# twndus/YelpRecommendation

Hardware: NVIDIA B200
Metric: ngcf_bpr_train_triples_per_sec (higher is better)
Workload: dtype f32

## Files before the change

yelprecommendation_b200/csrc/common.cuh:

```cuda
#pragma once
#include <cuda_runtime.h>
#include <cooperative_groups.h>
#include <stdint.h>
#include "../../include/yelprec_b200.h"

namespace cg = cooperative_groups;

#define YR_CHECK_LAUNCH()                                   \
  do {                                                      \
    cudaError_t e__ = cudaGetLastError();                   \
    if (e__ != cudaSuccess) return (int)e__;                \
  } while (0)

#define YR_CUDA(call)                                       \
  do {                                                      \
    cudaError_t e__ = (call);                               \
    if (e__ != cudaSuccess) return (int)e__;                \
  } while (0)

int yr_eval_exact_launch(const float* Uemb, int64_t nU, const float* Vt, int64_t ldt, int64_t nI, int d,
                         const int64_t* eval_uid, int64_t n_eval, const int32_t* mask_ptr,
                         const int32_t* mask_idx, const int32_t* act_ptr, const int32_t* act_idx,
                         const int32_t* act_nuniq, const double* inv_log2, int K, int64_t* topk_out,
                         float* topk_score, double* user_metrics, int32_t* err, const int32_t* row_list,
                         const int32_t* n_rows_dev, yr_stream stream, void* ws = nullptr, size_t ws_bytes = 0);
int yr_eval_reduce_launch(const double* user_metrics, const int32_t* act_ptr, const int32_t* act_nuniq,
                          int64_t n_eval, double* metric_sums, yr_stream stream);

int yr_ngcf_dense_fwd_tc_launch_d(int d, const float* E, const float* LE, const float* W1, const float* W2, float slope,
                                  int64_t n, float* Eout, cudaStream_t s, const int32_t* row_list = nullptr,
                                  const int32_t* row_count = nullptr, int64_t row_cap = 0, int reserve_sms = 0);
int yr_ngcf_dense_bwd_tc_launch(int d, const float* E, const float* LE, const float* En, const float* Gn, const float* W1,
                                const float* W2, float slope, int64_t n, float* G, float* T, float* ws, int* n_parts,
                                cudaStream_t s, const int32_t* row_list = nullptr, const int32_t* row_count = nullptr,
                                int64_t row_cap = 0, int reserve_sms = 0);
int yr_spmm_csr_rows(const yr_csr* A, int d, const float* X, float* Y, const int32_t* row_flag, cudaStream_t s);

namespace yr {

constexpr int kWarp = 32;
constexpr unsigned kFull = 0xffffffffu;

__device__ __forceinline__ float warp_sum(float v) {
#pragma unroll
  for (int o = 16; o > 0; o >>= 1) v += __shfl_xor_sync(kFull, v, o);
  return v;
}
__device__ __forceinline__ double warp_sum_d(double v) {
#pragma unroll
  for (int o = 16; o > 0; o >>= 1) v += __shfl_xor_sync(kFull, v, o);
  return v;
}

__device__ __forceinline__ void grid_sync(cg::grid_group& grid) {
  __syncwarp();
  grid.sync();
  __syncwarp();
}
// ... 181 lines not shown
```

yelprecommendation_b200/csrc/ngcf.cu:

```cuda
#include <stdlib.h>
#include "common.cuh"

namespace yr {

__device__ __forceinline__ void fma2(float2& acc, float a, const float2 b) { acc = __ffma2_rn(make_float2(a, a), b, acc); }

template <int D>
struct DenseCfg {
  static constexpr int kThreads = 256;
  static constexpr int kColGroups = D / 4;
  static constexpr int kRowGroups = kThreads / kColGroups;
  static constexpr int TM = 4 * kRowGroups;
  static constexpr int RO = D / kRowGroups;
  static constexpr size_t kSmemFwd = (size_t)(2 * D * TM + 2 * D * D) * sizeof(float);
  static constexpr size_t kSmemBwd = (size_t)(3 * TM * D + 2 * D * D) * sizeof(float);
  static_assert(D == 32 || D == 64 || D == 128, "dense transforms: D in {32, 64, 128}");
};

template <int D>
__global__ void __launch_bounds__(256)
ngcf_dense_fwd_kernel(const float* __restrict__ E, const float* __restrict__ LE,
                      const float* __restrict__ W1, const float* __restrict__ W2, float slope,
                      int64_t n, float* __restrict__ Eout) {
  using C = DenseCfg<D>;
// ... 436 lines not shown
                                 float slope, float* E_next, int dense_mode, yr_stream stream) {
  if (!E || !LE || !W1 || !W2 || !E_next || n < 0 || !mode_ok(dense_mode)) return YR_ERR_BAD_ARG;
  if (d != 32 && d != 64 && d != 128) return YR_ERR_BAD_DIM;
  if (n == 0) return YR_OK;
  if (fwd_tc(dense_mode) && (d == 64 || d == 128))
    return yr_ngcf_dense_fwd_tc_launch_d(d, E, LE, W1, W2, slope, n, E_next, (cudaStream_t)stream, nullptr, nullptr, 0,
                                         reserve_of(dense_mode));
  switch (d) {
    case 32: return dense_fwd_fp32_launch<32>(n, E, LE, W1, W2, slope, E_next, (cudaStream_t)stream);
    case 64: return dense_fwd_fp32_launch<64>(n, E, LE, W1, W2, slope, E_next, (cudaStream_t)stream);
    default: return dense_fwd_fp32_launch<128>(n, E, LE, W1, W2, slope, E_next, (cudaStream_t)stream);
  }
}

extern "C" int yr_ngcf_layer_fwd(const yr_csr* L, int d, const float* E, const float* W1, const float* W2,
                                 float slope, float* E_next, float* LE_save, int dense_mode, yr_stream stream) {
  if (!L || !E || !W1 || !W2 || !E_next || !LE_save || L->n_rows <= 0 || !mode_ok(dense_mode)) return YR_ERR_BAD_ARG;
  if (d != 32 && d != 64 && d != 128) return YR_ERR_BAD_DIM;
  int rc = yr_spmm_csr(L, d, E, LE_save, 0, stream);
  if (rc) return rc;
  return yr_ngcf_dense_fwd(d, L->n_rows, E, LE_save, W1, W2, slope, E_next, dense_mode, stream);
}

extern "C" size_t yr_ngcf_layer_bwd_ws_bytes(int d) {
  return (size_t)yr_sm_count() * kBwdCtasPerSm * 2 * (size_t)d * d * sizeof(float);
}

static int dense_bwd_launch(int d, int64_t n, const float* E, const float* LE, const float* E_next, const float* G_next,
                            const float* W1, const float* W2, float slope, float* G, float* T, void* ws, size_t ws_bytes,
                            int dense_mode, cudaStream_t s, int* n_parts) {
  if (!E || !LE || !E_next || !G_next || !W1 || !W2 || !G || !T || !ws || n <= 0 || !mode_ok(dense_mode)) return YR_ERR_BAD_ARG;
  if (d != 32 && d != 64 && d != 128) return YR_ERR_BAD_DIM;
  if (ws_bytes < yr_ngcf_layer_bwd_ws_bytes(d)) return YR_ERR_WORKSPACE;
  if (bwd_tc(dense_mode) && (d == 64 || d == 128))
    return yr_ngcf_dense_bwd_tc_launch(d, E, LE, E_next, G_next, W1, W2, slope, n, G, T, (float*)ws, n_parts, s, nullptr, nullptr,
                                       0, reserve_of(dense_mode));
  switch (d) {
    case 32: return dense_bwd_fp32_launch<32>(n, E, LE, E_next, G_next, W1, W2, slope, G, T, (float*)ws, s, n_parts);
    case 64: return dense_bwd_fp32_launch<64>(n, E, LE, E_next, G_next, W1, W2, slope, G, T, (float*)ws, s, n_parts);
    default: return dense_bwd_fp32_launch<128>(n, E, LE, E_next, G_next, W1, W2, slope, G, T, (float*)ws, s, n_parts);
  }
}

static int dense_bwd_reduce(int d, const void* ws, int n_parts, float* dW1, float* dW2, cudaStream_t s) {
  const int len = 2 * d * d;
  reduce_partials_kernel<<<(len + 31) / 32, 256, 0, s>>>((const float*)ws, n_parts, len, dW1, dW2, d * d);
  YR_CHECK_LAUNCH();
  return YR_OK;
}

extern "C" int yr_ngcf_dense_bwd(int d, int64_t n, const float* E, const float* LE, const float* E_next,
                                 const float* G_next, const float* W1, const float* W2, float slope,
                                 float* G, float* T, float* dW1, float* dW2, void* ws, size_t ws_bytes,
                                 int dense_mode, yr_stream stream) {
  if (!dW1 || !dW2) return YR_ERR_BAD_ARG;
  int parts = 0;
  int rc = dense_bwd_launch(d, n, E, LE, E_next, G_next, W1, W2, slope, G, T, ws, ws_bytes, dense_mode, (cudaStream_t)stream,
                            &parts);
  if (rc) return rc;
// ... 42 lines not shown
    float4 t[VPT];
#pragma unroll
    for (int v = 0; v < VPT; ++v)
      t[v] = len ? reinterpret_cast<const float4*>(T + (int64_t)row * D)[sl * VPT + v] : make_float4(0.f, 0.f, 0.f, 0.f);
    for (int j0 = 0; j0 < maxlen; j0 += LPR) {
      const int j = j0 + sl;
      const int cc = (j < len) ? __ldg(A.col + s0 + j) : -1;
      const float aa = (j < len) ? __ldg(A.val + s0 + j) : 0.f;
      for (int q = 0; q < LPR && j0 + q < maxlen; ++q) {
        const int cq = __shfl_sync(kFull, cc, q, LPR);
        const float a = __shfl_sync(kFull, aa, q, LPR);
        if (cq >= 0) {
#pragma unroll
          for (int v = 0; v < VPT; ++v)
            atomicAdd(reinterpret_cast<float4*>(G + (int64_t)cq * D) + sl * VPT + v,
                      make_float4(a * t[v].x, a * t[v].y, a * t[v].z, a * t[v].w));
        }
      }
    }
  }
}
}

struct SideStream { cudaStream_t stream; cudaEvent_t fork, join; };
static SideStream* side_stream() {
  static SideStream pool[64];
  static int state[64];
  const char* e = getenv("YR_NGCF_SIDE_STREAM");
  if (e && e[0] == '0') return nullptr;
  int dev = 0;
  if (cudaGetDevice(&dev) != cudaSuccess || dev < 0 || dev >= 64) return nullptr;
  if (state[dev] == 0) {
    SideStream& x = pool[dev];
    const bool ok = cudaStreamCreateWithFlags(&x.stream, cudaStreamNonBlocking) == cudaSuccess &&
                    cudaEventCreateWithFlags(&x.fork, cudaEventDisableTiming) == cudaSuccess &&
                    cudaEventCreateWithFlags(&x.join, cudaEventDisableTiming) == cudaSuccess;
    state[dev] = ok ? 1 : -1;
  }
  return state[dev] == 1 ? &pool[dev] : nullptr;
}

static int rows_reduce(const yr_ngcf_state* st, int l, int parts, cudaStream_t s, SideStream* side);

static int ngcf_layer_bwd_rows(const yr_ngcf_state* st, int l, float slope, cudaStream_t s, SideStream* side) {
  const int d = st->d;
  using C = DenseCfg<64>;
  if (d != 64) return YR_ERR_BAD_DIM;
  if (bwd_tc(st->dense_mode) && st->row_list_cap >= 16384) {
    int parts = 0;
    int rc = yr_ngcf_dense_bwd_tc_launch(d, st->E[l], st->LE[l], st->E[l + 1], st->G[l + 1], st->W1[l], st->W2[l], slope,
                                         st->nU + st->nI, st->G[l], st->T, (float*)st->ws, &parts, s, st->row_list,
                                         st->row_count, st->row_list_cap);
    if (rc) return rc;
    rc = rows_reduce(st, l, parts, s, side);
    if (rc) return rc;
    const int64_t blocks_tc = ((int64_t)st->L.n_chunks + 15) / 16;
    spmm_scatter_rows_kernel<64><<<(unsigned)blocks_tc, 256, 0, s>>>(st->L, st->row_flag, st->T, st->G[l]);
    YR_CHECK_LAUNCH();
    return YR_OK;
  }
  int64_t grid = (st->row_list_cap + C::TM - 1) / C::TM;
  const int64_t cap = (int64_t)yr_sm_count() * kBwdCtasPerSm;
  if (grid > cap) grid = cap;
  if (grid < 1) grid = 1;
  static AttrOnce attr;
  { int rc_ = attr.set(ngcf_dense_bwd_kernel<64>, (int)C::kSmemBwd); if (rc_) return rc_; }
  ngcf_dense_bwd_kernel<64><<<(unsigned)grid, C::kThreads, C::kSmemBwd, s>>>(
      st->E[l], st->LE[l], st->E[l + 1], st->G[l + 1], st->W1[l], st->W2[l], slope, st->nU + st->nI, st->G[l], st->T,
      (float*)st->ws, st->row_list, st->row_count);
  YR_CHECK_LAUNCH();
  int rc = rows_reduce(st, l, (int)grid, s, side);
  if (rc) return rc;
  const int wpb = 8, cpw = 2;
  int64_t blocks = ((int64_t)st->L.n_chunks + wpb * cpw - 1) / (wpb * cpw);
  spmm_scatter_rows_kernel<64><<<(unsigned)blocks, 256, 0, s>>>(st->L, st->row_flag, st->T, st->G[l]);
// ... 153 lines not shown
}

static int train_step_body(const yr_ngcf_state* st, const yr_opt* opt, float slope,
                           const int64_t* uid, const int64_t* pos, const int64_t* neg, int64_t B,
                           float* step_loss, int prefix_done, yr_stream stream, bool* rows_armed) {
  int rc = ngcf_state_ok(st);
  if (rc) return rc;
  if (prefix_done < 0 || prefix_done > st->n_layers) return YR_ERR_BAD_ARG;
  if (!opt || !uid || !pos || !neg || B <= 0 || yr_csr_ok(&st->LT) || !st->T ||
      !st->E_dev || !st->G_dev || !st->ws || !st->loss)
    return YR_ERR_BAD_ARG;
  if (opt->kind < YR_OPT_SGD || opt->kind > YR_OPT_ADAMW) return YR_ERR_BAD_OPT;
  const int L = st->n_layers, d = st->d;
  const int64_t n = st->nU + st->nI;
  cudaStream_t s = (cudaStream_t)stream;
  SideStream* side = side_stream();
  for (int l = 0; l <= L; ++l)
    if (!st->G[l]) return YR_ERR_BAD_ARG;
  cudaStream_t ms = side ? side->stream : s;
  if (side) {
    YR_CUDA(cudaEventRecord(side->fork, s));
    YR_CUDA(cudaStreamWaitEvent(side->stream, side->fork, 0));
  }
  for (int l = 0; l <= L; ++l) YR_CUDA(cudaMemsetAsync(st->G[l], 0, sizeof(float) * (size_t)n * d, ms));
  const bool rows_path = st->row_flag && st->row_list && st->row_count && st->row_list_cap >= 3 * B && d == 64 &&
                         st->top_rows_mode != 0;
  if (rows_path) {
    touched_rows_kernel<<<(unsigned)((3 * B + 255) / 256), 256, 0, ms>>>(uid, pos, neg, B, st->nU, st->nI, st->row_flag,
                                                                        st->row_list, st->row_count);
    YR_CHECK_LAUNCH();
    *rows_armed = true;
  }
  if (side) YR_CUDA(cudaEventRecord(side->join, side->stream));
  if (rows_path && fwd_tc(st->dense_mode)) {
    for (int l = (prefix_done < L - 1 ? prefix_done : L - 1); l + 1 < L; ++l) {
      rc = yr_ngcf_layer_fwd(&st->L, d, st->E[l], st->W1[l], st->W2[l], slope, st->E[l + 1], st->LE[l], st->dense_mode,
                           stream);
      if (rc) return rc;
    }
    if (side) YR_CUDA(cudaStreamWaitEvent(s, side->join, 0));
    rc = yr_spmm_csr_rows(&st->L, d, st->E[L - 1], st->LE[L - 1], st->row_flag, s);
    if (rc) return rc;
    rc = yr_ngcf_dense_fwd_tc_launch_d(d, st->E[L - 1], st->LE[L - 1], st->W1[L - 1], st->W2[L - 1], slope, n, st->E[L], s,
                                       st->row_list, st->row_count, 3 * B);
    if (rc) return rc;
  } else {
    for (int l = prefix_done; l < L; ++l) {
      rc = yr_ngcf_layer_fwd(&st->L, d, st->E[l], st->W1[l], st->W2[l], slope, st->E[l + 1], st->LE[l], st->dense_mode,
                           stream);
      if (rc) return rc;
    }
  }
  if (side) YR_CUDA(cudaStreamWaitEvent(s, side->join, 0));
  rc = yr_ngcf_tail(st->E_dev, st->G_dev, L, st->nU, st->nI, d, uid, pos, neg, B, nullptr, nullptr, st->loss,
                    step_loss, st->err, stream);
  if (rc) return rc;
  bool reduce_pending = false;
  for (int l = L - 1; l >= 0; --l) {
    if (!st->dW1[l] || !st->dW2[l]) return YR_ERR_BAD_ARG;
    if (rows_path && l == L - 1) {
      rc = ngcf_layer_bwd_rows(st, l, slope, s, side);
      if (rc) return rc;
      reduce_pending = side != nullptr;
      cudaStream_t us = s;
      if (side) {
        YR_CUDA(cudaStreamWaitEvent(s, side->join, 0));
        reduce_pending = false;
        YR_CUDA(cudaEventRecord(side->fork, s));
        YR_CUDA(cudaStreamWaitEvent(side->stream, side->fork, 0));
        us = side->stream;
      }
      untouch_rows_kernel<<<(unsigned)((3 * B + 255) / 256), 256, 0, us>>>(st->row_flag, st->row_list, st->row_count);
      YR_CHECK_LAUNCH();
      YR_CUDA(cudaMemsetAsync(st->row_count, 0, sizeof(int32_t), us));
      *rows_armed = false;
      continue;
    }
    if (side && reduce_pending) { YR_CUDA(cudaStreamWaitEvent(s, side->join, 0)); reduce_pending = false; }
    int parts = 0;
    rc = dense_bwd_launch(d, n, st->E[l], st->LE[l], st->E[l + 1], st->G[l + 1], st->W1[l], st->W2[l], slope, st->G[l],
                          st->T, st->ws, st->ws_bytes, st->dense_mode, s, &parts);
    if (rc) return rc;
    if (side) {
      YR_CUDA(cudaEventRecord(side->fork, s));
      YR_CUDA(cudaStreamWaitEvent(side->stream, side->fork, 0));
      rc = dense_bwd_reduce(d, st->ws, parts, st->dW1[l], st->dW2[l], side->stream);
      if (rc) return rc;
      YR_CUDA(cudaEventRecord(side->join, side->stream));
      reduce_pending = true;
    } else {
      rc = dense_bwd_reduce(d, st->ws, parts, st->dW1[l], st->dW2[l], s);
      if (rc) return rc;
    }
    rc = yr_spmm_csr(&st->LT, d, st->T, st->G[l], 1, stream);
    if (rc) return rc;
  }
  if (side && reduce_pending) YR_CUDA(cudaStreamWaitEvent(s, side->join, 0));
  float *pp[2 * YR_NGCF_MAX_LAYERS + 1], *gg[2 * YR_NGCF_MAX_LAYERS + 1], *mm[2 * YR_NGCF_MAX_LAYERS + 1],
      *vv[2 * YR_NGCF_MAX_LAYERS + 1];
  int64_t nn[2 * YR_NGCF_MAX_LAYERS + 1];
  int cnt = 0;
  pp[cnt] = st->E[0]; gg[cnt] = st->G[0]; mm[cnt] = st->mE; vv[cnt] = st->vE; nn[cnt++] = n * d;
  for (int l = 0; l < L; ++l) {
    pp[cnt] = st->W1[l]; gg[cnt] = st->dW1[l]; mm[cnt] = st->mW1[l]; vv[cnt] = st->vW1[l]; nn[cnt++] = (int64_t)d * d;
// ... 39 lines not shown
```

yelprecommendation_b200/csrc/ngcf_tc.cu:

```cuda
#include <stdlib.h>
#include "tc_common.cuh"

namespace yr {

constexpr int kFwdThreads = 416;
constexpr int kFwdTM = 128;

template <int D>
struct FwdTc {
  static_assert(D == 64 || D == 128, "tensor-core forward: d in {64, 128}");
  static constexpr bool kBRes = (D == 64);
  static constexpr int kSlabs = D / 32;
  static constexpr uint32_t kABytes = 128 * 128;
  static constexpr uint32_t kBBytes = D * 128;
  static constexpr uint32_t kStage = 2 * kABytes + (kBRes ? 0u : 2 * kBBytes);
  static constexpr int kNst = kBRes ? 4 : 3;
  static constexpr uint32_t kRing = kNst * kStage;
  static constexpr uint32_t kBResBytes = kBRes ? (uint32_t)(2 * kSlabs * 2) * kBBytes : 0u;
  static constexpr uint32_t kEpiOff = kRing + kBResBytes;
  static constexpr uint32_t kEpiBytes = 4 * 32 * 256;
  static constexpr uint32_t kBarOff = kEpiOff + kEpiBytes;
  static constexpr size_t kSmem = (size_t)kBarOff + 256 + 1024;
  static constexpr uint32_t kTmemCols = 4 * D;
  static constexpr size_t kWsBytes = (size_t)(2 * kSlabs) * 2 * kBBytes;
// ... 7 lines not shown
               "l"(src), "r"(bytes), "r"(s2u(bar))
               : "memory");
}

template <int D>
__global__ void __launch_bounds__(256)
ngcf_split_weights_kernel(const float* __restrict__ W1, const float* __restrict__ W2, unsigned char* __restrict__ ws) {
  using C = FwdTc<D>;
  const int total = 2 * D * (D / 4);
  for (int idx = blockIdx.x * blockDim.x + threadIdx.x; idx < total; idx += gridDim.x * blockDim.x) {
    const int X = idx / (D * (D / 4)), rem = idx % (D * (D / 4));
    const int o = rem / (D / 4), c4 = rem % (D / 4), j = c4 >> 3, c = c4 & 7;
    float4 hi, lo;
    split4(__ldg(reinterpret_cast<const float4*>((X ? W2 : W1) + o * D) + c4), hi, lo);
    unsigned char* blk = ws + (size_t)(j * 2 + X) * 2 * C::kBBytes;
    const uint32_t off = sw_off(D, o, c);
    *reinterpret_cast<float4*>(blk + off) = hi;
    *reinterpret_cast<float4*>(blk + C::kBBytes + off) = lo;
  }
}

template <int D>
__global__ void __launch_bounds__(kFwdThreads, 1)
ngcf_dense_fwd_tc_kernel(const float* __restrict__ E, const float* __restrict__ LE, const float* __restrict__ W1,
                         const float* __restrict__ W2, const unsigned char* __restrict__ wsplit, float slope, int64_t n,
                         float* __restrict__ Eout, const int32_t* __restrict__ row_list,
                         const int32_t* __restrict__ row_count) {
  using C = FwdTc<D>;
  constexpr int kSlabs = C::kSlabs, kNst = C::kNst;
  constexpr uint32_t kABytes = C::kABytes, kBBytes = C::kBBytes, kStage = C::kStage;
  if (row_list) n = *row_count;
  extern __shared__ __align__(16) unsigned char smem_raw[];
  unsigned char* smem = smem_raw + ((1024u - (s2u(smem_raw) & 1023u)) & 1023u);
  unsigned char* ring = smem;
  unsigned char* bres = smem + C::kRing;
  uint64_t* bars = reinterpret_cast<uint64_t*>(smem + C::kBarOff);
  uint64_t* full = bars; uint64_t* empty = bars + kNst; uint64_t* d_full = bars + 2 * kNst; uint64_t* d_empty = d_full + 2;
  uint32_t* tmem_slot = reinterpret_cast<uint32_t*>(d_empty + 2);

  const int tid = threadIdx.x, lane = tid & 31, warp = tid >> 5;
  const int64_t n_tiles = (n + kFwdTM - 1) / kFwdTM;
  const int64_t my_tiles = (int64_t)blockIdx.x < n_tiles ? (n_tiles - blockIdx.x + gridDim.x - 1) / gridDim.x : 0;

  if (tid == 0) {
    for (int s = 0; s < kNst; ++s) { mbar_init(full + s, 1); mbar_init(empty + s, 1); }
    for (int a = 0; a < 2; ++a) { mbar_init(d_full + a, 1); mbar_init(d_empty + a, 128); }
    asm volatile("fence.mbarrier_init.release.cluster;" ::: "memory");
  }
  if (warp == 12) tmem_alloc(tmem_slot, C::kTmemCols);
  if constexpr (C::kBRes) {
    for (int idx = tid; idx < D * (D / 4); idx += kFwdThreads) {
      const int o = idx / (D / 4), c4 = idx % (D / 4), j = c4 >> 3, c = c4 & 7;
      const uint32_t off = sw_off(D, o, c);
      float4 hi, lo;
      split4(__ldg(reinterpret_cast<const float4*>(W1 + o * D) + c4), hi, lo);
      *reinterpret_cast<float4*>(bres + (size_t)((0 * kSlabs + j) * 2 + 0) * kBBytes + off) = hi;
      *reinterpret_cast<float4*>(bres + (size_t)((0 * kSlabs + j) * 2 + 1) * kBBytes + off) = lo;
      split4(__ldg(reinterpret_cast<const float4*>(W2 + o * D) + c4), hi, lo);
      *reinterpret_cast<float4*>(bres + (size_t)((1 * kSlabs + j) * 2 + 0) * kBBytes + off) = hi;
      *reinterpret_cast<float4*>(bres + (size_t)((1 * kSlabs + j) * 2 + 1) * kBBytes + off) = lo;
    }
  }
  asm volatile("fence.proxy.async.shared::cta;" ::: "memory");
  tc_fence_before();
  __syncthreads();
  tc_fence_after();
  const uint32_t tmem_base = *tmem_slot;
  const uint32_t idesc = (1u << 4) | (2u << 7) | (2u << 10) | ((uint32_t)(D >> 3) << 17) | ((uint32_t)(128 >> 4) << 24);

  if (warp < 8) {
    const int c = tid & 7, rb = tid >> 3;
    const int64_t n_items = my_tiles * kSlabs;
    uint32_t s = 0, ph = 0;
    constexpr int kPfTiles = 1;
    auto prefetch_tile = [&](int64_t ti) {
      if (row_list || ti >= my_tiles) return;
      const int64_t r0 = (blockIdx.x + ti * gridDim.x) * kFwdTM;
      const int64_t rows = (n - r0) < kFwdTM ? (n - r0) : kFwdTM;
      l2_prefetch_bulk(E + r0 * D, (uint32_t)(rows * D * 4));
      l2_prefetch_bulk(LE + r0 * D, (uint32_t)(rows * D * 4));
    };
    auto issue = [&](int64_t item, float4 (&e)[4], float4 (&le)[4]) {
      const int64_t tile = blockIdx.x + (item / kSlabs) * gridDim.x;
      const int j = (int)(item % kSlabs);
#pragma unroll
      for (int i = 0; i < 4; ++i) {
// ... 83 lines not shown
            o.z = o.z > 0.f ? o.z : o.z * slope; o.w = o.w > 0.f ? o.w : o.w * slope;
            *reinterpret_cast<float4*>(stg + lane * 256 + (((8 * half + k) ^ (lane & 15)) << 4)) = o;
          }
        }
        __syncwarp();
        {
#pragma unroll 4
          for (int i = 0; i < 16; ++i) {
            const int rr = 2 * i + (lane >> 4), c4 = lane & 15;
            const int64_t q = q0 + rr;
            const float4 o = *reinterpret_cast<const float4*>(stg + rr * 256 + ((c4 ^ (rr & 15)) << 4));
            if (q < n) {
              const int64_t row = row_list ? (int64_t)__ldg(row_list + q) : q;
              reinterpret_cast<float4*>(Eout + row * D + 64 * h)[c4] = o;
            }
          }
        }
        __syncwarp();
      }
      if (++acc == 2) { acc = 0; aph ^= 1; }
    }
  } else if (lane == 0) {
    uint32_t s = 0, ph = 0, acc = 0, aph = 0;
    for (int64_t t = 0; t < my_tiles; ++t) {
      mbar_wait(d_empty + acc, aph ^ 1);
      tc_fence_after();
      const uint32_t tacc = tmem_base + acc * 2 * D;
      uint32_t first_big = 1, first_small = 1;
#pragma unroll 1
      for (int jx = 0; jx < 2 * kSlabs; ++jx) {
        const int j = jx >> 1, X = jx & 1;
        mbar_wait(full + s, ph);
        tc_fence_after();
        const uint32_t a_hi = s2u(ring + (size_t)s * kStage), a_lo = a_hi + kABytes;
        const uint32_t b_hi = C::kBRes ? s2u(bres + (size_t)((X * kSlabs + j) * 2) * kBBytes) : a_hi + 2 * kABytes;
        const uint32_t b_lo = b_hi + kBBytes;
        const uint32_t pa[3] = {a_lo, a_hi, a_hi};
        const uint32_t pb[3] = {b_hi, b_lo, b_hi};
#pragma unroll
        for (int p = 0; p < 3; ++p) {
          const uint64_t ad = sw128_desc(pa[p]), bd = sw128_desc(pb[p]);
#pragma unroll
          for (int ks = 0; ks < 4; ++ks) {
            if (p < 2) { umma_tf32(tacc + D, ad + 2 * ks, bd + 2 * ks, idesc, first_small ? 0u : 1u); first_small = 0; }
            else       { umma_tf32(tacc, ad + 2 * ks, bd + 2 * ks, idesc, first_big ? 0u : 1u); first_big = 0; }
          }
        }
        umma_commit(empty + s);
        if (++s == (uint32_t)kNst) { s = 0; ph ^= 1; }
      }
      umma_commit(d_full + acc);
      if (++acc == 2) { acc = 0; aph ^= 1; }
    }
  }
  tc_fence_before();
  __syncthreads();
  if (warp == 12) tmem_dealloc(tmem_base, C::kTmemCols);
}

}

using namespace yr;

template <int D>
static int fwd_tc_launch(const float* E, const float* LE, const float* W1, const float* W2, float slope, int64_t n,
                         float* Eout, cudaStream_t s, const int32_t* row_list, const int32_t* row_count, int64_t row_cap,
                         int reserve_sms) {
  using C = FwdTc<D>;
  static yr::AttrOnce attr;
  { int rc_ = attr.set(ngcf_dense_fwd_tc_kernel<D>, (int)C::kSmem); if (rc_) return rc_; }
  const int64_t n_tiles = ((row_list ? row_cap : n) + kFwdTM - 1) / kFwdTM;
  int64_t grid = yr_sm_count() - reserve_sms;
  if (grid > n_tiles) grid = n_tiles;
  if (grid < 1) grid = 1;
  unsigned char* ws = nullptr;
  if (!C::kBRes) {
    static bool pool_set[64] = {};
    int dev = 0;
    YR_CUDA(cudaGetDevice(&dev));
    if (dev >= 0 && dev < 64 && !pool_set[dev]) {
      cudaMemPool_t pool;
      unsigned long long keep = 64ull << 20;
      YR_CUDA(cudaDeviceGetDefaultMemPool(&pool, dev));
      YR_CUDA(cudaMemPoolSetAttribute(pool, cudaMemPoolAttrReleaseThreshold, &keep));
      pool_set[dev] = true;
    }
    YR_CUDA(cudaMallocAsync((void**)&ws, C::kWsBytes, s));
    ngcf_split_weights_kernel<D><<<16, 256, 0, s>>>(W1, W2, ws);
  }
  ngcf_dense_fwd_tc_kernel<D><<<(unsigned)grid, kFwdThreads, C::kSmem, s>>>(E, LE, W1, W2, ws, slope, n, Eout, row_list,
                                                                            row_count);
  cudaError_t e = cudaGetLastError();
  if (ws) cudaFreeAsync(ws, s);
  return e == cudaSuccess ? YR_OK : (int)e;
}

int yr_ngcf_dense_fwd_tc_launch_d(int d, const float* E, const float* LE, const float* W1, const float* W2, float slope,
                                  int64_t n, float* Eout, cudaStream_t s, const int32_t* row_list,
                                  const int32_t* row_count, int64_t row_cap, int reserve_sms) {
  if (d == 64) return fwd_tc_launch<64>(E, LE, W1, W2, slope, n, Eout, s, row_list, row_count, row_cap, reserve_sms);
  if (d == 128) return fwd_tc_launch<128>(E, LE, W1, W2, slope, n, Eout, s, row_list, row_count, row_cap, reserve_sms);
  return YR_ERR_BAD_ARG;
}
```

yelprecommendation_b200/csrc/ngcf_tc_bwd.cu:

```cuda
#include <stdlib.h>
#include "tc_common.cuh"

namespace yr {

constexpr int kBwdThreads = 416;
constexpr int kBwdTM = 128;
constexpr int kFlushTiles = 4;

__device__ __forceinline__ uint32_t mn_off(int mn, int k, uint32_t lbo, uint32_t sbo) {
  return (uint32_t)(k >> 2) * sbo + (uint32_t)(mn >> 5) * lbo + (uint32_t)(k & 3) * 128u +
         ((((uint32_t)(mn & 31) >> 3) ^ (uint32_t)(k & 3)) << 5) + (uint32_t)(mn & 7) * 4u;
}
__device__ __forceinline__ uint64_t mn_desc(uint32_t smem_addr, uint32_t lbo, uint32_t sbo) {
  uint64_t d = 0;
  d |= (uint64_t)((smem_addr & 0x3FFFFu) >> 4);
  d |= (uint64_t)((lbo >> 4) & 0x3FFFu) << 16;
  d |= (uint64_t)((sbo >> 4) & 0x3FFFu) << 32;
  d |= (uint64_t)1 << 46;
  d |= (uint64_t)1 << 61;
  return d;
}
__device__ __forceinline__ void mbar_expect_tx_b(uint64_t* bar, uint32_t bytes) {
  asm volatile("mbarrier.expect_tx.relaxed.cta.shared::cta.b64 [%0], %1;" ::"r"(s2u(bar)), "r"(bytes) : "memory");
}
// ... 35 lines not shown
  for (int idx = blockIdx.x * blockDim.x + threadIdx.x; idx < total; idx += gridDim.x * blockDim.x) {
    const int X = idx / (D * (D / 4)), rem = idx % (D * (D / 4));
    const int o = rem / (D / 4), c4 = rem % (D / 4), j = o >> 5, k = o & 31;
    float4 hi, lo;
    split4(__ldg(reinterpret_cast<const float4*>((X ? W2 : W1) + o * D) + c4), hi, lo);
    const int pair = C::kXG == 2 ? X : 0;
    const int mn = C::kXG == 2 ? 4 * c4 : X * D + 4 * c4;
    unsigned char* blk = ws + (size_t)(j * C::kXG + pair) * C::kPair;
    const uint32_t off = mn_off(mn, k, C::kLbo, C::kSboW);
    *reinterpret_cast<float4*>(blk + off) = hi;
    *reinterpret_cast<float4*>(blk + C::kBlk + off) = lo;
  }
}

template <int D>
__global__ void __launch_bounds__(kBwdThreads, 1)
ngcf_dense_bwd_tc_kernel(const float* __restrict__ E, const float* __restrict__ LE, const float* __restrict__ Enext,
                         const float* __restrict__ Gnext, const unsigned char* __restrict__ wsplit, float slope, int64_t n,
                         float* __restrict__ G, float* __restrict__ T, float* __restrict__ ws,
                         const int32_t* __restrict__ row_list, const int32_t* __restrict__ row_count) {
  using C = BwdTc<D>;
  constexpr int TM = kBwdTM, kNst = C::kNst, kXG = C::kXG, kSlabs = C::kSlabs, kHalves = C::kHalves, kItems = C::kItems;
  constexpr uint32_t kBlk = C::kBlk, kPair = C::kPair, kStage = C::kStage;
  if (row_list) n = *row_count;
  extern __shared__ __align__(16) unsigned char smem_raw[];
  unsigned char* smem = smem_raw + ((1024u - (s2u(smem_raw) & 1023u)) & 1023u);
  unsigned char* ring = smem;
  uint64_t* bars = reinterpret_cast<uint64_t*>(smem + C::kBarOff);
  uint64_t* full = bars; uint64_t* empty = bars + kNst; uint64_t* d1_full = bars + 2 * kNst; uint64_t* d1_empty = d1_full + 2;
  uint64_t* d2_full = d1_full + 4; uint64_t* d2_empty = d1_full + 5;
  uint32_t* tmem_slot = reinterpret_cast<uint32_t*>(d1_full + 6);
  constexpr int kAcc = C::kAcc;

  const int tid = threadIdx.x, lane = tid & 31, warp = tid >> 5;
  const int64_t n_tiles = (n + TM - 1) / TM;
  const int64_t my_tiles = (int64_t)blockIdx.x < n_tiles ? (n_tiles - blockIdx.x + gridDim.x - 1) / gridDim.x : 0;

  if (tid == 0) {
    for (int s = 0; s < kNst; ++s) { mbar_init(full + s, 1); mbar_init(empty + s, 1); }
    for (int a = 0; a < 2; ++a) { mbar_init(d1_full + a, 1); mbar_init(d1_empty + a, 128); }
    mbar_init(d2_full, 1); mbar_init(d2_empty, 128);
    asm volatile("fence.mbarrier_init.release.cluster;" ::: "memory");
  }
  if (warp == 12) tmem_alloc(tmem_slot, C::kTmemCols);
  tc_fence_before();
  __syncthreads();
// ... 258 lines not shown
              umma_tf32(tmem_base + C::kColG2 + x * 128, ad, bd, idesc2, (first2 && p == 0 && ks == 0) ? 0u : 1u);
            }
          }
        }
        first2 = 0;
        umma_commit(empty + s);
        if (++s == (uint32_t)kNst) { s = 0; ph ^= 1; }
      }
      if ((t + 1) % kFlushTiles == 0 || t + 1 == my_tiles) umma_commit(d2_full);
    }
  }
  tc_fence_before();
  __syncthreads();
  if (warp == 12) tmem_dealloc(tmem_base, C::kTmemCols);
}

}

using namespace yr;

template <int D>
static int bwd_tc_launch(const float* E, const float* LE, const float* En, const float* Gn, const float* W1, const float* W2,
                         float slope, int64_t n, float* G, float* T, float* ws, int* n_parts, cudaStream_t s,
                         const int32_t* row_list, const int32_t* row_count, int64_t row_cap, int reserve_sms) {
  using C = BwdTc<D>;
  static yr::AttrOnce attr;
  { int rc_ = attr.set(ngcf_dense_bwd_tc_kernel<D>, (int)C::kSmem); if (rc_) return rc_; }
  const int64_t n_tiles = ((row_list ? row_cap : n) + kBwdTM - 1) / kBwdTM;
  const int64_t sms = yr_sm_count();
  int64_t grid = sms - reserve_sms;
  if (grid > n_tiles) grid = n_tiles;
  if (grid < 1) grid = 1;
  unsigned char* wsplit = reinterpret_cast<unsigned char*>(ws) + (size_t)sms * 2 * D * D * sizeof(float);
  ngcf_split_weights_bwd_kernel<D><<<16, 256, 0, s>>>(W1, W2, wsplit);
  YR_CHECK_LAUNCH();
  ngcf_dense_bwd_tc_kernel<D><<<(unsigned)grid, kBwdThreads, C::kSmem, s>>>(E, LE, En, Gn, wsplit, slope, n, G, T, ws, row_list,
                                                                            row_count);
  YR_CHECK_LAUNCH();
  *n_parts = (int)grid;
  return YR_OK;
}

int yr_ngcf_dense_bwd_tc_launch(int d, const float* E, const float* LE, const float* En, const float* Gn, const float* W1,
                                const float* W2, float slope, int64_t n, float* G, float* T, float* ws, int* n_parts,
                                cudaStream_t s, const int32_t* row_list, const int32_t* row_count, int64_t row_cap,
                                int reserve_sms) {
  if (d == 64) return bwd_tc_launch<64>(E, LE, En, Gn, W1, W2, slope, n, G, T, ws, n_parts, s, row_list, row_count, row_cap, reserve_sms);
  if (d == 128) return bwd_tc_launch<128>(E, LE, En, Gn, W1, W2, slope, n, G, T, ws, n_parts, s, row_list, row_count, row_cap, reserve_sms);
  return YR_ERR_BAD_DIM;
}
```

yelprecommendation_b200/csrc/tc_common.cuh:

```cuda
#pragma once
#include <cuda.h>
#include "common.cuh"

namespace yr {

__device__ __forceinline__ uint32_t s2u(const void* p) { return (uint32_t)__cvta_generic_to_shared(p); }

__device__ __forceinline__ void mbar_init(uint64_t* bar, int count) {
  asm volatile("mbarrier.init.shared::cta.b64 [%0], %1;" ::"r"(s2u(bar)), "r"(count) : "memory");
}
__device__ __forceinline__ void mbar_expect_tx(uint64_t* bar, uint32_t bytes) {
  asm volatile("mbarrier.arrive.expect_tx.shared::cta.b64 _, [%0], %1;" ::"r"(s2u(bar)), "r"(bytes) : "memory");
}
__device__ __forceinline__ void mbar_arrive(uint64_t* bar) {
  asm volatile("mbarrier.arrive.shared::cta.b64 _, [%0];" ::"r"(s2u(bar)) : "memory");
}
__device__ __forceinline__ void mbar_wait(uint64_t* bar, uint32_t parity) {
  asm volatile(
      "{\n\t.reg .pred p;\n\t"
      "TC_WAIT:\n\t"
      "mbarrier.try_wait.parity.shared::cta.b64 p, [%0], %1;\n\t"
      "@p bra TC_DONE;\n\t"
      "bra TC_WAIT;\n\t"
      "TC_DONE:\n\t}" ::"r"(s2u(bar)),
      "r"(parity)
      : "memory");
}
__device__ __forceinline__ void tma_load_2d(void* dst, const CUtensorMap* map, int c0, int c1, uint64_t* bar) {
  asm volatile(
      "cp.async.bulk.tensor.2d.shared::cluster.global.tile.mbarrier::complete_tx::bytes [%0], [%1, {%3, %4}], [%2];"
      ::"r"(s2u(dst)), "l"(map), "r"(s2u(bar)), "r"(c0), "r"(c1)
      : "memory");
}
__device__ __forceinline__ void l2_prefetch_bulk(const void* src, uint32_t bytes) {
  asm volatile("cp.async.bulk.prefetch.L2.global [%0], %1;" ::"l"(src), "r"(bytes) : "memory");
}
__device__ __forceinline__ void tmem_alloc(uint32_t* dst_smem, uint32_t ncols) {
  asm volatile("tcgen05.alloc.cta_group::1.sync.aligned.shared::cta.b32 [%0], %1;" ::"r"(s2u(dst_smem)), "r"(ncols)
               : "memory");
  asm volatile("tcgen05.relinquish_alloc_permit.cta_group::1.sync.aligned;" ::: "memory");
}
__device__ __forceinline__ void tmem_dealloc(uint32_t taddr, uint32_t ncols) {
  asm volatile("tcgen05.dealloc.cta_group::1.sync.aligned.b32 %0, %1;" ::"r"(taddr), "r"(ncols) : "memory");
}
__device__ __forceinline__ void tc_fence_before() { asm volatile("tcgen05.fence::before_thread_sync;" ::: "memory"); }
__device__ __forceinline__ void tc_fence_after() { asm volatile("tcgen05.fence::after_thread_sync;" ::: "memory"); }
__device__ __forceinline__ void umma_tf32(uint32_t tmem_d, uint64_t adesc, uint64_t bdesc, uint32_t idesc,
                                          uint32_t accumulate) {
  asm volatile(
      "{\n\t.reg .pred p;\n\t"
      "setp.ne.b32 p, %4, 0;\n\t"
      "tcgen05.mma.cta_group::1.kind::tf32 [%0], %1, %2, %3, p;\n\t}" ::"r"(tmem_d),
      "l"(adesc), "l"(bdesc), "r"(idesc), "r"(accumulate)
      : "memory");
}
__device__ __forceinline__ void umma_commit(uint64_t* bar) {
  asm volatile("tcgen05.commit.cta_group::1.mbarrier::arrive::one.shared::cluster.b64 [%0];" ::"r"(s2u(bar))
               : "memory");
// ... 67 lines not shown
```

Baseline: 3.975 million.

## Pre-split NGCF weights once per step and launch dense TC kernels with PDL

Splits W1/W2 into hi/lo TF32 swizzled form once per training step per layer on the side stream, storing the result in the extended workspace. The forward and backward tensor-core kernels then reuse it instead of re-splitting per launch: the forward kernel bulk-copies the pre-split weights into shared memory via TMA with an mbarrier rather than computing the split in every CTA. Both kernels are launched with programmatic dependent launch and call griddepcontrol.wait, so their launch and prologue can overlap the tail of the previous kernel. This adds workspace, an extra side-stream event and cross-stream synchronisation, plus a risk of stale weights if the optimizer updates W before the split is consumed.

```diff
diff --git a/yelprecommendation_b200/csrc/common.cuh b/yelprecommendation_b200/csrc/common.cuh
--- a/yelprecommendation_b200/csrc/common.cuh
+++ b/yelprecommendation_b200/csrc/common.cuh
@@ -29,11 +29,16 @@
 
 int yr_ngcf_dense_fwd_tc_launch_d(int d, const float* E, const float* LE, const float* W1, const float* W2, float slope,
                                   int64_t n, float* Eout, cudaStream_t s, const int32_t* row_list = nullptr,
-                                  const int32_t* row_count = nullptr, int64_t row_cap = 0, int reserve_sms = 0);
+                                  const int32_t* row_count = nullptr, int64_t row_cap = 0, int reserve_sms = 0,
+                                  const unsigned char* wsplit = nullptr);
 int yr_ngcf_dense_bwd_tc_launch(int d, const float* E, const float* LE, const float* En, const float* Gn, const float* W1,
                                 const float* W2, float slope, int64_t n, float* G, float* T, float* ws, int* n_parts,
                                 cudaStream_t s, const int32_t* row_list = nullptr, const int32_t* row_count = nullptr,
-                                int64_t row_cap = 0, int reserve_sms = 0);
+                                int64_t row_cap = 0, int reserve_sms = 0, const unsigned char* wsplit = nullptr);
+size_t yr_ngcf_fwd_tc_split_bytes(int d);
+size_t yr_ngcf_bwd_tc_split_bytes(int d);
+int yr_ngcf_fwd_tc_split(int d, const float* W1, const float* W2, unsigned char* ws, cudaStream_t s);
+int yr_ngcf_bwd_tc_split(int d, const float* W1, const float* W2, unsigned char* ws, cudaStream_t s);
 int yr_spmm_csr_rows(const yr_csr* A, int d, const float* X, float* Y, const int32_t* row_flag, cudaStream_t s);
 
 namespace yr {
diff --git a/yelprecommendation_b200/csrc/ngcf.cu b/yelprecommendation_b200/csrc/ngcf.cu
--- a/yelprecommendation_b200/csrc/ngcf.cu
+++ b/yelprecommendation_b200/csrc/ngcf.cu
@@ -482,19 +482,28 @@
   return yr_ngcf_dense_fwd(d, L->n_rows, E, LE_save, W1, W2, slope, E_next, dense_mode, stream);
 }
 
+static size_t bwd_partials_bytes(int d) { return (size_t)yr_sm_count() * kBwdCtasPerSm * 2 * (size_t)d * d * sizeof(float); }
+static size_t step_split_bytes(int d) { return d == 64 ? yr_ngcf_fwd_tc_split_bytes(d) + yr_ngcf_bwd_tc_split_bytes(d) : 0; }
+static unsigned char* step_split_fwd(const yr_ngcf_state* st, int l) {
+  return (unsigned char*)st->ws + bwd_partials_bytes(st->d) + (size_t)l * step_split_bytes(st->d);
+}
+static unsigned char* step_split_bwd(const yr_ngcf_state* st, int l) {
+  return step_split_fwd(st, l) + yr_ngcf_fwd_tc_split_bytes(st->d);
+}
+
 extern "C" size_t yr_ngcf_layer_bwd_ws_bytes(int d) {
-  return (size_t)yr_sm_count() * kBwdCtasPerSm * 2 * (size_t)d * d * sizeof(float);
+  return bwd_partials_bytes(d) + YR_NGCF_MAX_LAYERS * step_split_bytes(d);
 }
 
 static int dense_bwd_launch(int d, int64_t n, const float* E, const float* LE, const float* E_next, const float* G_next,
                             const float* W1, const float* W2, float slope, float* G, float* T, void* ws, size_t ws_bytes,
-                            int dense_mode, cudaStream_t s, int* n_parts) {
+                            int dense_mode, cudaStream_t s, int* n_parts, const unsigned char* wsplit = nullptr) {
   if (!E || !LE || !E_next || !G_next || !W1 || !W2 || !G || !T || !ws || n <= 0 || !mode_ok(dense_mode)) return YR_ERR_BAD_ARG;
   if (d != 32 && d != 64 && d != 128) return YR_ERR_BAD_DIM;
-  if (ws_bytes < yr_ngcf_layer_bwd_ws_bytes(d)) return YR_ERR_WORKSPACE;
+  if (ws_bytes < bwd_partials_bytes(d)) return YR_ERR_WORKSPACE;
   if (bwd_tc(dense_mode) && (d == 64 || d == 128))
     return yr_ngcf_dense_bwd_tc_launch(d, E, LE, E_next, G_next, W1, W2, slope, n, G, T, (float*)ws, n_parts, s, nullptr, nullptr,
-                                       0, reserve_of(dense_mode));
+                                       0, reserve_of(dense_mode), wsplit);
   switch (d) {
     case 32: return dense_bwd_fp32_launch<32>(n, E, LE, E_next, G_next, W1, W2, slope, G, T, (float*)ws, s, n_parts);
     case 64: return dense_bwd_fp32_launch<64>(n, E, LE, E_next, G_next, W1, W2, slope, G, T, (float*)ws, s, n_parts);
@@ -583,7 +592,7 @@
 }
 }
 
-struct SideStream { cudaStream_t stream; cudaEvent_t fork, join; };
+struct SideStream { cudaStream_t stream; cudaEvent_t fork, join, split; };
 static SideStream* side_stream() {
   static SideStream pool[64];
   static int state[64];
@@ -595,7 +604,8 @@
     SideStream& x = pool[dev];
     const bool ok = cudaStreamCreateWithFlags(&x.stream, cudaStreamNonBlocking) == cudaSuccess &&
                     cudaEventCreateWithFlags(&x.fork, cudaEventDisableTiming) == cudaSuccess &&
-                    cudaEventCreateWithFlags(&x.join, cudaEventDisableTiming) == cudaSuccess;
+                    cudaEventCreateWithFlags(&x.join, cudaEventDisableTiming) == cudaSuccess &&
+                    cudaEventCreateWithFlags(&x.split, cudaEventDisableTiming) == cudaSuccess;
     state[dev] = ok ? 1 : -1;
   }
   return state[dev] == 1 ? &pool[dev] : nullptr;
@@ -611,7 +621,7 @@
     int parts = 0;
     int rc = yr_ngcf_dense_bwd_tc_launch(d, st->E[l], st->LE[l], st->E[l + 1], st->G[l + 1], st->W1[l], st->W2[l], slope,
                                          st->nU + st->nI, st->G[l], st->T, (float*)st->ws, &parts, s, st->row_list,
-                                         st->row_count, st->row_list_cap);
+                                         st->row_count, st->row_list_cap, 0, step_split_bwd(st, l));
     if (rc) return rc;
     rc = rows_reduce(st, l, parts, s, side);
     if (rc) return rc;
@@ -811,6 +821,33 @@
     YR_CUDA(cudaEventRecord(side->fork, s));
     YR_CUDA(cudaStreamWaitEvent(side->stream, side->fork, 0));
   }
+  const bool tc_split = d == 64 && fwd_tc(st->dense_mode);
+  if (tc_split) {
+    if (st->ws_bytes < yr_ngcf_layer_bwd_ws_bytes(d)) return YR_ERR_WORKSPACE;
+    for (int l = 0; l < L; ++l) {
+      rc = yr_ngcf_fwd_tc_split(d, st->W1[l], st->W2[l], step_split_fwd(st, l), ms);
+      if (!rc && bwd_tc(st->dense_mode)) rc = yr_ngcf_bwd_tc_split(d, st->W1[l], st->W2[l], step_split_bwd(st, l), ms);
+      if (rc) return rc;
+    }
+    if (side) YR_CUDA(cudaEventRecord(side->split, side->stream));
+  }
+  bool split_waited = !side || !tc_split;
+  auto split_ready = [&]() -> int {
+    if (!split_waited) YR_CUDA(cudaStreamWaitEvent(s, side->split, 0));
+    split_waited = true;
+    return YR_OK;
+  };
+  auto layer_fwd = [&](int l) -> int {
+    if (!tc_split)
+      return yr_ngcf_layer_fwd(&st->L, d, st->E[l], st->W1[l], st->W2[l], slope, st->E[l + 1], st->LE[l], st->dense_mode,
+                               stream);
+    int rc_ = yr_spmm_csr(&st->L, d, st->E[l], st->LE[l], 0, stream);
+    if (!rc_) rc_ = split_ready();
+    if (!rc_)
+      rc_ = yr_ngcf_dense_fwd_tc_launch_d(d, st->E[l], st->LE[l], st->W1[l], st->W2[l], slope, n, st->E[l + 1], s, nullptr,
+                                          nullptr, 0, reserve_of(st->dense_mode), step_split_fwd(st, l));
+    return rc_;
+  };
   for (int l = 0; l <= L; ++l) YR_CUDA(cudaMemsetAsync(st->G[l], 0, sizeof(float) * (size_t)n * d, ms));
   const bool rows_path = st->row_flag && st->row_list && st->row_count && st->row_list_cap >= 3 * B && d == 64 &&
                          st->top_rows_mode != 0;
@@ -823,20 +860,19 @@
   if (side) YR_CUDA(cudaEventRecord(side->join, side->stream));
   if (rows_path && fwd_tc(st->dense_mode)) {
     for (int l = (prefix_done < L - 1 ? prefix_done : L - 1); l + 1 < L; ++l) {
-      rc = yr_ngcf_layer_fwd(&st->L, d, st->E[l], st->W1[l], st->W2[l], slope, st->E[l + 1], st->LE[l], st->dense_mode,
-                           stream);
+      rc = layer_fwd(l);
       if (rc) return rc;
     }
     if (side) YR_CUDA(cudaStreamWaitEvent(s, side->join, 0));
+    split_waited = true;
     rc = yr_spmm_csr_rows(&st->L, d, st->E[L - 1], st->LE[L - 1], st->row_flag, s);
     if (rc) return rc;
     rc = yr_ngcf_dense_fwd_tc_launch_d(d, st->E[L - 1], st->LE[L - 1], st->W1[L - 1], st->W2[L - 1], slope, n, st->E[L], s,
-                                       st->row_list, st->row_count, 3 * B);
+                                       st->row_list, st->row_count, 3 * B, 0, tc_split ? step_split_fwd(st, L - 1) : nullptr);
     if (rc) return rc;
   } else {
     for (int l = prefix_done; l < L; ++l) {
-      rc = yr_ngcf_layer_fwd(&st->L, d, st->E[l], st->W1[l], st->W2[l], slope, st->E[l + 1], st->LE[l], st->dense_mode,
-                           stream);
+      rc = layer_fwd(l);
       if (rc) return rc;
     }
   }
@@ -868,7 +904,7 @@
     if (side && reduce_pending) { YR_CUDA(cudaStreamWaitEvent(s, side->join, 0)); reduce_pending = false; }
     int parts = 0;
     rc = dense_bwd_launch(d, n, st->E[l], st->LE[l], st->E[l + 1], st->G[l + 1], st->W1[l], st->W2[l], slope, st->G[l],
-                          st->T, st->ws, st->ws_bytes, st->dense_mode, s, &parts);
+                          st->T, st->ws, st->ws_bytes, st->dense_mode, s, &parts, tc_split ? step_split_bwd(st, l) : nullptr);
     if (rc) return rc;
     if (side) {
       YR_CUDA(cudaEventRecord(side->fork, s));
diff --git a/yelprecommendation_b200/csrc/ngcf_tc.cu b/yelprecommendation_b200/csrc/ngcf_tc.cu
--- a/yelprecommendation_b200/csrc/ngcf_tc.cu
+++ b/yelprecommendation_b200/csrc/ngcf_tc.cu
@@ -53,13 +53,14 @@
 
 template <int D>
 __global__ void __launch_bounds__(kFwdThreads, 1)
-ngcf_dense_fwd_tc_kernel(const float* __restrict__ E, const float* __restrict__ LE, const float* __restrict__ W1,
-                         const float* __restrict__ W2, const unsigned char* __restrict__ wsplit, float slope, int64_t n,
+ngcf_dense_fwd_tc_kernel(const float* __restrict__ E, const float* __restrict__ LE,
+                         const unsigned char* __restrict__ wsplit, float slope, int64_t n,
                          float* __restrict__ Eout, const int32_t* __restrict__ row_list,
                          const int32_t* __restrict__ row_count) {
   using C = FwdTc<D>;
   constexpr int kSlabs = C::kSlabs, kNst = C::kNst;
   constexpr uint32_t kABytes = C::kABytes, kBBytes = C::kBBytes, kStage = C::kStage;
+  grid_dep_wait();
   if (row_list) n = *row_count;
   extern __shared__ __align__(16) unsigned char smem_raw[];
   unsigned char* smem = smem_raw + ((1024u - (s2u(smem_raw) & 1023u)) & 1023u);
@@ -67,7 +68,8 @@
   unsigned char* bres = smem + C::kRing;
   uint64_t* bars = reinterpret_cast<uint64_t*>(smem + C::kBarOff);
   uint64_t* full = bars; uint64_t* empty = bars + kNst; uint64_t* d_full = bars + 2 * kNst; uint64_t* d_empty = d_full + 2;
-  uint32_t* tmem_slot = reinterpret_cast<uint32_t*>(d_empty + 2);
+  uint64_t* w_full = d_empty + 2;
+  uint32_t* tmem_slot = reinterpret_cast<uint32_t*>(d_empty + 3);
 
   const int tid = threadIdx.x, lane = tid & 31, warp = tid >> 5;
   const int64_t n_tiles = (n + kFwdTM - 1) / kFwdTM;
@@ -76,23 +78,14 @@
   if (tid == 0) {
     for (int s = 0; s < kNst; ++s) { mbar_init(full + s, 1); mbar_init(empty + s, 1); }
     for (int a = 0; a < 2; ++a) { mbar_init(d_full + a, 1); mbar_init(d_empty + a, 128); }
+    mbar_init(w_full, 1);
     asm volatile("fence.mbarrier_init.release.cluster;" ::: "memory");
+    if constexpr (C::kBRes) {
+      mbar_expect_tx(w_full, C::kBResBytes);
+      bulk_g2s_tc(bres, wsplit, C::kBResBytes, w_full);
+    }
   }
   if (warp == 12) tmem_alloc(tmem_slot, C::kTmemCols);
-  if constexpr (C::kBRes) {
-    for (int idx = tid; idx < D * (D / 4); idx += kFwdThreads) {
-      const int o = idx / (D / 4), c4 = idx % (D / 4), j = c4 >> 3, c = c4 & 7;
-      const uint32_t off = sw_off(D, o, c);
-      float4 hi, lo;
-      split4(__ldg(reinterpret_cast<const float4*>(W1 + o * D) + c4), hi, lo);
-      *reinterpret_cast<float4*>(bres + (size_t)((0 * kSlabs + j) * 2 + 0) * kBBytes + off) = hi;
-      *reinterpret_cast<float4*>(bres + (size_t)((0 * kSlabs + j) * 2 + 1) * kBBytes + off) = lo;
-      split4(__ldg(reinterpret_cast<const float4*>(W2 + o * D) + c4), hi, lo);
-      *reinterpret_cast<float4*>(bres + (size_t)((1 * kSlabs + j) * 2 + 0) * kBBytes + off) = hi;
-      *reinterpret_cast<float4*>(bres + (size_t)((1 * kSlabs + j) * 2 + 1) * kBBytes + off) = lo;
-    }
-  }
-  asm volatile("fence.proxy.async.shared::cta;" ::: "memory");
   tc_fence_before();
   __syncthreads();
   tc_fence_after();
@@ -222,6 +215,7 @@
     }
   } else if (lane == 0) {
     uint32_t s = 0, ph = 0, acc = 0, aph = 0;
+    if constexpr (C::kBRes) mbar_wait(w_full, 0);
     for (int64_t t = 0; t < my_tiles; ++t) {
       mbar_wait(d_empty + acc, aph ^ 1);
       tc_fence_after();
@@ -233,7 +227,7 @@
         mbar_wait(full + s, ph);
         tc_fence_after();
         const uint32_t a_hi = s2u(ring + (size_t)s * kStage), a_lo = a_hi + kABytes;
-        const uint32_t b_hi = C::kBRes ? s2u(bres + (size_t)((X * kSlabs + j) * 2) * kBBytes) : a_hi + 2 * kABytes;
+        const uint32_t b_hi = C::kBRes ? s2u(bres + (size_t)(jx * 2) * kBBytes) : a_hi + 2 * kABytes;
         const uint32_t b_lo = b_hi + kBBytes;
         const uint32_t pa[3] = {a_lo, a_hi, a_hi};
         const uint32_t pb[3] = {b_hi, b_lo, b_hi};
@@ -265,7 +259,7 @@
 template <int D>
 static int fwd_tc_launch(const float* E, const float* LE, const float* W1, const float* W2, float slope, int64_t n,
                          float* Eout, cudaStream_t s, const int32_t* row_list, const int32_t* row_count, int64_t row_cap,
-                         int reserve_sms) {
+                         int reserve_sms, const unsigned char* wsplit) {
   using C = FwdTc<D>;
   static yr::AttrOnce attr;
   { int rc_ = attr.set(ngcf_dense_fwd_tc_kernel<D>, (int)C::kSmem); if (rc_) return rc_; }
@@ -274,7 +268,7 @@
   if (grid > n_tiles) grid = n_tiles;
   if (grid < 1) grid = 1;
   unsigned char* ws = nullptr;
-  if (!C::kBRes) {
+  if (!wsplit) {
     static bool pool_set[64] = {};
     int dev = 0;
     YR_CUDA(cudaGetDevice(&dev));
@@ -287,18 +281,31 @@
     }
     YR_CUDA(cudaMallocAsync((void**)&ws, C::kWsBytes, s));
     ngcf_split_weights_kernel<D><<<16, 256, 0, s>>>(W1, W2, ws);
+    wsplit = ws;
   }
-  ngcf_dense_fwd_tc_kernel<D><<<(unsigned)grid, kFwdThreads, C::kSmem, s>>>(E, LE, W1, W2, ws, slope, n, Eout, row_list,
-                                                                            row_count);
-  cudaError_t e = cudaGetLastError();
+  cudaError_t e = launch_pdl(ngcf_dense_fwd_tc_kernel<D>, (unsigned)grid, kFwdThreads, C::kSmem, s, E, LE, wsplit, slope, n,
+                             Eout, row_list, row_count);
+  if (e == cudaSuccess) e = cudaGetLastError();
   if (ws) cudaFreeAsync(ws, s);
   return e == cudaSuccess ? YR_OK : (int)e;
 }
 
 int yr_ngcf_dense_fwd_tc_launch_d(int d, const float* E, const float* LE, const float* W1, const float* W2, float slope,
                                   int64_t n, float* Eout, cudaStream_t s, const int32_t* row_list,
-                                  const int32_t* row_count, int64_t row_cap, int reserve_sms) {
-  if (d == 64) return fwd_tc_launch<64>(E, LE, W1, W2, slope, n, Eout, s, row_list, row_count, row_cap, reserve_sms);
-  if (d == 128) return fwd_tc_launch<128>(E, LE, W1, W2, slope, n, Eout, s, row_list, row_count, row_cap, reserve_sms);
+                                  const int32_t* row_count, int64_t row_cap, int reserve_sms, const unsigned char* wsplit) {
+  if (d == 64) return fwd_tc_launch<64>(E, LE, W1, W2, slope, n, Eout, s, row_list, row_count, row_cap, reserve_sms, wsplit);
+  if (d == 128) return fwd_tc_launch<128>(E, LE, W1, W2, slope, n, Eout, s, row_list, row_count, row_cap, reserve_sms, wsplit);
   return YR_ERR_BAD_ARG;
 }
+
+size_t yr_ngcf_fwd_tc_split_bytes(int d) {
+  return d == 64 ? FwdTc<64>::kWsBytes : d == 128 ? FwdTc<128>::kWsBytes : 0;
+}
+
+int yr_ngcf_fwd_tc_split(int d, const float* W1, const float* W2, unsigned char* ws, cudaStream_t s) {
+  if (d == 64) ngcf_split_weights_kernel<64><<<16, 256, 0, s>>>(W1, W2, ws);
+  else if (d == 128) ngcf_split_weights_kernel<128><<<16, 256, 0, s>>>(W1, W2, ws);
+  else return YR_ERR_BAD_ARG;
+  YR_CHECK_LAUNCH();
+  return YR_OK;
+}
diff --git a/yelprecommendation_b200/csrc/ngcf_tc_bwd.cu b/yelprecommendation_b200/csrc/ngcf_tc_bwd.cu
--- a/yelprecommendation_b200/csrc/ngcf_tc_bwd.cu
+++ b/yelprecommendation_b200/csrc/ngcf_tc_bwd.cu
@@ -81,6 +81,7 @@
   using C = BwdTc<D>;
   constexpr int TM = kBwdTM, kNst = C::kNst, kXG = C::kXG, kSlabs = C::kSlabs, kHalves = C::kHalves, kItems = C::kItems;
   constexpr uint32_t kBlk = C::kBlk, kPair = C::kPair, kStage = C::kStage;
+  grid_dep_wait();
   if (row_list) n = *row_count;
   extern __shared__ __align__(16) unsigned char smem_raw[];
   unsigned char* smem = smem_raw + ((1024u - (s2u(smem_raw) & 1023u)) & 1023u);
@@ -385,7 +386,8 @@
 template <int D>
 static int bwd_tc_launch(const float* E, const float* LE, const float* En, const float* Gn, const float* W1, const float* W2,
                          float slope, int64_t n, float* G, float* T, float* ws, int* n_parts, cudaStream_t s,
-                         const int32_t* row_list, const int32_t* row_count, int64_t row_cap, int reserve_sms) {
+                         const int32_t* row_list, const int32_t* row_count, int64_t row_cap, int reserve_sms,
+                         const unsigned char* wsplit) {
   using C = BwdTc<D>;
   static yr::AttrOnce attr;
   { int rc_ = attr.set(ngcf_dense_bwd_tc_kernel<D>, (int)C::kSmem); if (rc_) return rc_; }
@@ -394,11 +396,15 @@
   int64_t grid = sms - reserve_sms;
   if (grid > n_tiles) grid = n_tiles;
   if (grid < 1) grid = 1;
-  unsigned char* wsplit = reinterpret_cast<unsigned char*>(ws) + (size_t)sms * 2 * D * D * sizeof(float);
-  ngcf_split_weights_bwd_kernel<D><<<16, 256, 0, s>>>(W1, W2, wsplit);
-  YR_CHECK_LAUNCH();
-  ngcf_dense_bwd_tc_kernel<D><<<(unsigned)grid, kBwdThreads, C::kSmem, s>>>(E, LE, En, Gn, wsplit, slope, n, G, T, ws, row_list,
-                                                                            row_count);
+  if (!wsplit) {
+    unsigned char* own = reinterpret_cast<unsigned char*>(ws) + (size_t)sms * 2 * D * D * sizeof(float);
+    ngcf_split_weights_bwd_kernel<D><<<16, 256, 0, s>>>(W1, W2, own);
+    YR_CHECK_LAUNCH();
+    wsplit = own;
+  }
+  const cudaError_t e = launch_pdl(ngcf_dense_bwd_tc_kernel<D>, (unsigned)grid, kBwdThreads, C::kSmem, s, E, LE, En, Gn, wsplit,
+                                   slope, n, G, T, ws, row_list, row_count);
+  if (e != cudaSuccess) return (int)e;
   YR_CHECK_LAUNCH();
   *n_parts = (int)grid;
   return YR_OK;
@@ -407,8 +413,20 @@
 int yr_ngcf_dense_bwd_tc_launch(int d, const float* E, const float* LE, const float* En, const float* Gn, const float* W1,
                                 const float* W2, float slope, int64_t n, float* G, float* T, float* ws, int* n_parts,
                                 cudaStream_t s, const int32_t* row_list, const int32_t* row_count, int64_t row_cap,
-                                int reserve_sms) {
-  if (d == 64) return bwd_tc_launch<64>(E, LE, En, Gn, W1, W2, slope, n, G, T, ws, n_parts, s, row_list, row_count, row_cap, reserve_sms);
-  if (d == 128) return bwd_tc_launch<128>(E, LE, En, Gn, W1, W2, slope, n, G, T, ws, n_parts, s, row_list, row_count, row_cap, reserve_sms);
+                                int reserve_sms, const unsigned char* wsplit) {
+  if (d == 64) return bwd_tc_launch<64>(E, LE, En, Gn, W1, W2, slope, n, G, T, ws, n_parts, s, row_list, row_count, row_cap, reserve_sms, wsplit);
+  if (d == 128) return bwd_tc_launch<128>(E, LE, En, Gn, W1, W2, slope, n, G, T, ws, n_parts, s, row_list, row_count, row_cap, reserve_sms, wsplit);
   return YR_ERR_BAD_DIM;
 }
+
+size_t yr_ngcf_bwd_tc_split_bytes(int d) {
+  return d == 64 ? BwdTc<64>::kWsplitBytes : d == 128 ? BwdTc<128>::kWsplitBytes : 0;
+}
+
+int yr_ngcf_bwd_tc_split(int d, const float* W1, const float* W2, unsigned char* ws, cudaStream_t s) {
+  if (d == 64) ngcf_split_weights_bwd_kernel<64><<<16, 256, 0, s>>>(W1, W2, ws);
+  else if (d == 128) ngcf_split_weights_bwd_kernel<128><<<16, 256, 0, s>>>(W1, W2, ws);
+  else return YR_ERR_BAD_DIM;
+  YR_CHECK_LAUNCH();
+  return YR_OK;
+}
diff --git a/yelprecommendation_b200/csrc/tc_common.cuh b/yelprecommendation_b200/csrc/tc_common.cuh
--- a/yelprecommendation_b200/csrc/tc_common.cuh
+++ b/yelprecommendation_b200/csrc/tc_common.cuh
@@ -34,6 +34,22 @@
 }
 __device__ __forceinline__ void l2_prefetch_bulk(const void* src, uint32_t bytes) {
   asm volatile("cp.async.bulk.prefetch.L2.global [%0], %1;" ::"l"(src), "r"(bytes) : "memory");
+}
+__device__ __forceinline__ void grid_dep_wait() { asm volatile("griddepcontrol.wait;" ::: "memory"); }
+template <typename... KArgs, typename... Args>
+static cudaError_t launch_pdl(void (*kernel)(KArgs...), unsigned grid, unsigned block, size_t smem, cudaStream_t s,
+                              Args... args) {
+  cudaLaunchConfig_t cfg = {};
+  cfg.gridDim = dim3(grid);
+  cfg.blockDim = dim3(block);
+  cfg.dynamicSmemBytes = smem;
+  cfg.stream = s;
+  cudaLaunchAttribute attr[1];
+  attr[0].id = cudaLaunchAttributeProgrammaticStreamSerialization;
+  attr[0].val.programmaticStreamSerializationAllowed = 1;
+  cfg.attrs = attr;
+  cfg.numAttrs = 1;
+  return cudaLaunchKernelEx(&cfg, kernel, static_cast<KArgs>(args)...);
 }
 __device__ __forceinline__ void tmem_alloc(uint32_t* dst_smem, uint32_t ncols) {
   asm volatile("tcgen05.alloc.cta_group::1.sync.aligned.shared::cta.b32 [%0], %1;" ::"r"(s2u(dst_smem)), "r"(ncols)
```

Result: no change. 3.946 million, median of 6 (-0.7%).
